# mike-gimelfarb/bboptpy

Measured on AMD Instinct MI355X. Metric: candidate-evals/sec, higher is better.
Workload: dtype f64; 1 GPU; ActiveCMAES n=128 np=4096 rosenbrock, 256 independent populations per GPU in lockstep; populations_per_gpu=256, n=128, np=4096, objective=rosenbrock

## Files before the change

bboptpy_amd/csrc/bbo_cma.hip:

```cpp
#include "bbo_cma_kernels.hpp"
#include "bbo_sep_kernels.hpp"
#include "bbo_eig_mw.hpp"

#include <algorithm>
#include <atomic>
#include <cmath>
#include <cstdlib>
#include <limits>

namespace bbo {

namespace {

enum { K_SAMPLE = 0, K_RANK, K_WHITEN, K_GRAM, K_PATHS, K_COV, K_EIGEN, K_POST, K_STOP, K_COUNT };
static const char *const K_NAMES[K_COUNT] = { "bbo:cma_sample_eval", "bbo:cma_rank", "bbo:cma_whiten", "bbo:cma_gram", "bbo:cma_paths", "bbo:cma_cov", "bbo:cma_eigen", "bbo:cma_post", "bbo:cma_history_stop" };

int pick_maxt(int ld)
{
    const int per_wave = ((ld >> 4) + 3) / 4;
    if (per_wave <= 1) return 1;
    if (per_wave <= 2) return 2;
    if (per_wave <= 4) return 4;
    return 8;
}
// ... 88 lines not shown

bool CmaEngine::mw_reserve(long workgroups)
{
    if (mw_reserved_ == workgroups) return true;
    mw_release();
    if (!MwBudget::get().reserve(params_.device, workgroups)) return false;
    mw_reserved_ = workgroups;
    return true;
}

void CmaEngine::mw_release()
{
    if (mw_reserved_ > 0) MwBudget::get().release(params_.device, mw_reserved_);
    mw_reserved_ = 0;
}

bool CmaEngine::mw_check_failed()
{
    if (!mw_launched_) return false;
    mw_launched_ = false;
    if (!*mw_fail_host_) return false;
    *mw_fail_host_ = 0;
    mw_disabled_ = true;
    mw_release();
    return true;
}

void CmaEngine::set_params(int np, double sigma, int mfev)
{
    params_.np = np;
    params_.sigma0 = sigma;
    params_.mfev = mfev;
    if (params_.bound) {
        params_.bound = 0;
        fprintf(stderr, "Warning [CMA]: box bounding is no longer enabled.\n");
    }
}

void CmaEngine::init(int n, const double *lower, const double *upper, const double *guess,
        const ObjectiveSpec &obj)
{
    const bool sep = params_.algo == BBO_ALGO_SEP_CMAES;
    if (sep)
        BBO_REQUIRE(n >= 1 && n <= 4096, "SepCMAES: dimension must be in [1, 4096]");
    else
        BBO_REQUIRE(n >= 1 && n <= EIG_NMAX, "dimension must be in [1, 512]");
    BBO_HIP(hipSetDevice(params_.device));
    obj_ = obj;
    const int P = params_.populations;
    const int lambda = params_.np;
    CmaConst &c = c_;
    c = CmaConst {};
    c.n = n;
    c.ld = round_up(n, 16);
    c.lambda = lambda;
    c.lambda_pad = round_up(lambda, 16);
    c.mu = lambda / 2;
    c.mu_pad = round_up(c.mu, 16);
    c.variant = sep ? 2 : params_.algo == BBO_ALGO_ACTIVE_CMAES ? 1 : 0;
    c.bound = params_.bound ? 1 : 0;
    c.lazy_isc = (!sep && !c.bound && c.ld > 16 && c.ld <= 256) ? 1 : 0;
    c.obj = obj.on_device() ? obj.builtin : OBJ_HOST;
    c.mfev = params_.mfev;
    c.mit = params_.mfev / lambda;
    c.npop = P;
    c.seed = params_.seed;
    c.tol = params_.tol;
    c.sigma0 = params_.sigma0;
    c.stop_off = 0;
    c.ftarget = -std::numeric_limits<double>::infinity();

    std::vector<double> w(c.mu);
    double sum = 0.;
    for (int i = 0; i < c.mu; i++) {
        w[i] = std::log(0.5 * (lambda + 1.)) - std::log(i + 1.);
        sum += w[i];
    }
    const double inv = 1. / sum;
    for (int i = 0; i < c.mu; i++) w[i] *= inv;
    double lenw = 0.;
    for (int i = 0; i < c.mu; i++) lenw = lenw + w[i] * w[i];
    c.mueff = 1. / lenw;

    c.chi = std::sqrt(n) * (1. - 1. / (4. * n) + 1. / (21. * n * n));
    c.cc = (4. + c.mueff / n) / (n + 4. + 2. * c.mueff / n);
    c.cs = (c.mueff + 2.) / (5. + n + c.mueff);
    c.c1 = 2. / ((1.3 + n) * (1.3 + n) + c.mueff);
    c.cmu = std::min(1. - c.c1,
            2. * (c.mueff - 2. + 1. / c.mueff) / ((2. + n) * (2. + n) + c.mueff));
    c.damps = 1. + c.cs + 2. * std::max(0., std::sqrt((c.mueff - 1.) / (n + 1.)) - 1.);
    c.hlen = 10 + (int) std::ceil((30. * n) / lambda);
    c.ik = (int) std::ceil(0.1 + lambda / 4.);
    c.eigenfreq = params_.eigenrate * lambda / (c.c1 + c.cmu) / n;
    c.cm = 1.;
    c.alphaold = 0.5;
    c.cneg = 0.;
    if (c.variant == 1) {
        const double ac = params_.alphacov;
        c.cc = (4. + 0. * c.mueff / n) / (n + 4. + 0. * 2. * c.mueff / n);
        c.cs = (c.mueff + 2.) / (3. + n + c.mueff);
        c.c1 = ac * std::min(1., lambda / 6.) / ((n + 1.3) * (n + 1.3) + c.mueff);
        c.cmu = 1. - c.c1;
        c.cmu = std::min(c.cmu,
                ac * (c.mueff - 2. + 1. / c.mueff) / ((2. + n) * (2. + n) + ac * c.mueff / 2.));
        c.cneg = (1. - c.cmu) * (ac / 8.) * c.mueff / (std::pow(n + 2., 1.5) + 2. * c.mueff);
        c.damps = 1. + c.cs + 2. * std::max(0., std::sqrt((c.mueff - 1.) / (n + 1.)) - 1.);
        c.eigenfreq = params_.eigenrate * (1. / (c.c1 + c.cmu + c.cneg)) / n;
    }

    if (sep) {
        c.cc = 4. / (n + 4.);
        c.cs = (c.mueff + 2.) / (3. + n + c.mueff);
        c.damps = 1. + c.cs + 2. * std::max(0., std::sqrt((c.mueff - 1.) / (n + 1.)) - 1.);
        c.ccov = 2. / ((n + std::sqrt(2.)) * (n + std::sqrt(2.)) * c.mueff);
        c.ccov += std::min(1., (2. * c.mueff - 1.) / ((n + 2.) * (n + 2.) + c.mueff))
                * (1. - 1. / c.mueff);
        if (params_.adjustlr) c.ccov *= ((n + 2.) / 3.);
    }

    c.rps = 64;
    while (c.rps > 16 && gram_lds_bytes(c.ld, c.rps) > GRAM_LDS_MAX) c.rps >>= 1;
    if (c.ld == 128) {
        int cap = 32;
        if (const char *e = std::getenv("BBO_GRAM_WANT")) cap = std::max(1, std::atoi(e));
        int want = std::max(1, std::min(cap, (512 + P - 1) / P));
        want = std::min(want, (c.lambda_pad + G128_CH - 1) / G128_CH);
        c.rps = ((c.lambda_pad + want - 1) / want + G128_CH - 1) / G128_CH * G128_CH;
    }
    c.splits = (c.lambda_pad + c.rps - 1) / c.rps;
    if (sep)
        c.splits = std::max(1, std::min(c.mu / 16, (1024 + P - 1) / P));

    const size_t ld = c.ld, ld2 = ld * ld;
    const bool same_shape = !sep && keep_bc_ && last_n_ == n && C_.count == P * ld2;
    X_.alloc((size_t) P * c.lambda_pad * ld);
    f_.alloc((size_t) P * c.lambda_pad);
    zn2_.alloc((size_t) P * c.lambda_pad);
    rank_.alloc((size_t) P * c.lambda_pad);
    order_.alloc((size_t) P * c.lambda_pad);
    xmean_.alloc(P * ld);
    xold_.alloc(P * ld);
    pc_.alloc(P * ld);
    ps_.alloc(P * ld);
    D_.alloc(P * ld);
    csep_.alloc(P * ld);
    if (!sep) {
        isc_.alloc(P * ld2);
        BDp_.alloc(P * ld2);
        ISp_.alloc(P * ld2);
    }
    S_.alloc((size_t) P * c.mu_pad);
    gram_part_.alloc((size_t) P * c.splits * (sep ? ld : ld2));
    mean_part_.alloc((size_t) P * c.splits * ld);
    hist_best_.alloc((size_t) P * c.hlen);
    hist_kth_.alloc((size_t) P * c.hlen);
    weights_.alloc(c.mu);
    weights_.upload(w.data(), c.mu);
    lower_.alloc(ld);
    upper_.alloc(ld);
    aux_.alloc(ld);
    scal_.alloc(P);
    zinject_.release();
    zrecord_.release();

    lower_h_.assign(ld, 0.);
    upper_h_.assign(ld, 0.);
    aux_h_.assign(ld, 0.);
    std::copy(lower, lower + n, lower_h_.begin());
    std::copy(upper, upper + n, upper_h_.begin());
    fill_objective_aux(obj.on_device() ? obj.builtin : -1, n, aux_h_.data());
    lower_.upload(lower_h_.data(), ld);
    upper_.upload(upper_h_.data(), ld);
    aux_.upload(aux_h_.data(), ld);

    std::vector<double> eye(sep ? 0 : P * ld2, 0.), ones(P * ld, 1.);
    csep_.upload(ones.data(), P * ld);
    if (!sep) {
    for (int p = 0; p < P; p++)
        for (int i = 0; i < n; i++) eye[p * ld2 + (size_t) i * ld + i] = 1.;
    if (same_shape) {
        std::vector<double> bm(P * ld2), cm(P * ld2);
        B_.download(bm.data(), P * ld2);
        C_.download(cm.data(), P * ld2);
        for (int p = 0; p < P; p++)
            for (int i = 0; i < n; i++) {
                bm[p * ld2 + (size_t) i * ld + i] = 1.;
                cm[p * ld2 + (size_t) i * ld + i] = 1.;
            }
        B_.upload(bm.data(), P * ld2);
        C_.upload(cm.data(), P * ld2);
    } else {
        B_.alloc(P * ld2);
        C_.alloc(P * ld2);
        B_.upload(eye.data(), P * ld2);
        C_.upload(eye.data(), P * ld2);
    }
    isc_.upload(eye.data(), P * ld2);
    }
    D_.upload(ones.data(), P * ld);
    keep_bc_ = !sep;
    last_n_ = n;

    std::vector<double> xm(P * ld, 0.);
    for (int p = 0; p < P; p++) std::copy(guess + (size_t) p * n, guess + (size_t) (p + 1) * n,
            xm.begin() + p * ld);
    xmean_.upload(xm.data(), P * ld);

    std::vector<CmaScal> sc(P);
    for (auto &s : sc) {
        std::memset(&s, 0, sizeof(s));
        s.sigma = params_.sigma0;
        s.fbest = -std::numeric_limits<double>::infinity();
        s.fworst = std::numeric_limits<double>::infinity();
        s.hist_head = -1;
        s.basis_ok = same_shape ? 0 : 1;
    }
    scal_.upload(sc.data(), P);
    basis_maybe_stale_ = same_shape;

    if (!sep) eig_work_.alloc((size_t) P * 4 * eig_slab((int) ld));

    CmaDev &d = d_;
    d = CmaDev {};
    d.X = X_.p; d.f = f_.p; d.rank = rank_.p; d.order = order_.p;
    d.xmean = xmean_.p; d.xold = xold_.p; d.pc = pc_.p; d.ps = ps_.p;
    d.C = C_.p; d.B = B_.p; d.D = D_.p; d.isc = isc_.p; d.BDp = BDp_.p; d.ISp = ISp_.p;
    d.S = S_.p; d.zn2 = zn2_.p; d.csep = csep_.p; d.gram_part = gram_part_.p; d.mean_part = mean_part_.p;
    d.hist_best = hist_best_.p; d.hist_kth = hist_kth_.p; d.eig_work = eig_work_.p;
    d.weights = weights_.p; d.lower = lower_.p; d.upper = upper_.p; d.aux = aux_.p;
    d.zinject = nullptr; d.zrecord = nullptr; d.scal = scal_.p;
    d.stamps = stamps_.p;
    d.mw_fail_host = mw_fail_host_;
    d.mw_fault = mw_fault_from_env();
    mw_release();

    c.honor_stop = 0;
    inited_ = true;
    if (!sep) {
        launch_post(2);
        BBO_HIP(hipGetLastError());
        BBO_HIP(hipStreamSynchronize(stream_));
    }
}

void CmaEngine::launch_post(int mode)
{
    const CmaConst &c = c_;
    if (c.ld <= 128) {
        const size_t lds = (size_t) (c.ld * (c.ld + 2) + c.ld) * sizeof(double);
        allow_lds((const void*) cma_post_mfma<1>, 140 * 1024);
        allow_lds((const void*) cma_post_mfma<4>, 140 * 1024);
        if (c.npop < 32)
            hipLaunchKernelGGL(cma_post_mfma<4>, dim3(c.npop, 4), dim3(256), lds, stream_, d_, c_,
                    mode);
        else
            hipLaunchKernelGGL(cma_post_mfma<1>, dim3(c.npop, 1), dim3(256), lds, stream_, d_, c_,
                    mode);
    } else {
        dim3 grid(c.ld / 16, c.ld / 16, c.npop);
        hipLaunchKernelGGL(cma_post, grid, dim3(256), 0, stream_, d_, c_, mode);
    }
}

void CmaEngine::launch_sample_eval()
{
    const CmaConst &c = c_;
    bool zn_valid = false;
    timer_.begin(stream_, K_SAMPLE);
    if (c.variant == 2) {
        const int per_pop = std::max(1, 4096 / c.npop);
        if (c.ld <= 256) {
            allow_lds((const void*) sep_sample_eval<16>, 128 * 1024);
            const size_t lds = (size_t) 16 * c.ld * sizeof(double);
            hipLaunchKernelGGL(sep_sample_eval<16>,
                    dim3(std::min((c.lambda_pad + 15) / 16, per_pop), c.npop), dim3(256), lds,
                    stream_, d_, c_);
        } else if (c.ld <= 2048) {
            const size_t lds = (size_t) 8 * c.ld * sizeof(double);
            const dim3 grid(std::min((c.lambda_pad + 7) / 8, per_pop), c.npop);
            if (c.n == c.ld && !c.bound && c.lambda == c.lambda_pad && !d_.zinject
                    && !d_.zrecord && !(d_.dbg & 256)) {
                if (sep_sum_objective(c.obj) && !(d_.dbg & 1048576)) {
                    const dim3 sgrid(std::min(c.lambda_pad / (4 * SEP_K), per_pop), c.npop);
#define BBO_SEP_SUM(NCV, OBJV) hipLaunchKernelGGL((sep_sample_sum<256, NCV, OBJV>), sgrid, dim3(256), 0, stream_, d_, c_)
#define BBO_SEP_SUM_OBJ(NCV) \
                    switch (c.obj) { \
                    case OBJ_SPHERE: BBO_SEP_SUM(NCV, OBJ_SPHERE); break; \
                    case OBJ_ELLIPSOID: BBO_SEP_SUM(NCV, OBJ_ELLIPSOID); break; \
                    case OBJ_RASTRIGIN: BBO_SEP_SUM(NCV, OBJ_RASTRIGIN); break; \
                    case OBJ_CIGAR: BBO_SEP_SUM(NCV, OBJ_CIGAR); break; \
                    case OBJ_DISCUS: BBO_SEP_SUM(NCV, OBJ_DISCUS); break; \
                    default: BBO_SEP_SUM(NCV, OBJ_DIFFPOW); break; \
                    }
                    if (c.ld == 1024 && c.obj != OBJ_RASTRIGIN && c.obj != OBJ_DIFFPOW) { BBO_SEP_SUM_OBJ(4) }
                    else { BBO_SEP_SUM_OBJ(0) }
#undef BBO_SEP_SUM_OBJ
#undef BBO_SEP_SUM
                } else {
                    allow_lds((const void*) sep_sample_eval<64, 512, true>, 140 * 1024);
                    hipLaunchKernelGGL((sep_sample_eval<64, 512, true>), grid, dim3(512), lds,
                            stream_, d_, c_);
                }
            } else {
                allow_lds((const void*) sep_sample_eval<64, 512>, 140 * 1024);
                hipLaunchKernelGGL((sep_sample_eval<64, 512>), grid, dim3(512), lds, stream_,
                        d_, c_);
            }
        } else {
            allow_lds((const void*) sep_sample_eval<64>, 140 * 1024);
            const size_t lds = (size_t) 4 * c.ld * sizeof(double);
            hipLaunchKernelGGL(sep_sample_eval<64>,
                    dim3(std::min((c.lambda_pad + 3) / 4, per_pop), c.npop), dim3(256), lds,
                    stream_, d_, c_);
        }
        timer_.end(stream_);
        BBO_HIP(hipGetLastError());
        c_.use_zn = 0;
        return;
    }
    if (c.ld == 128 && (long) c.npop * c.lambda_pad >= sample128_min_rows_
            && (c.obj < 0 || frag_objective_ok(c.obj))) {
        int rw = (int) (((long) c.npop * c.lambda_pad / 256 + 127) / 128) * 128;
        rw = std::max(128, std::min(4096, rw));
        allow_lds((const void*) cma_sample_eval128, 128 * 1024);
        dim3 grid((c.lambda_pad + rw - 1) / rw, c.npop);
        const int full = (c.n == 128 && !c.bound && c.lambda == c.lambda_pad && !d_.zinject
                && !d_.zrecord && !(d_.dbg & 256)) ? 1 : 0;
        hipLaunchKernelGGL(cma_sample_eval128, grid, dim3(512), 128 * 1024, stream_, d_, c_, rw,
                full);
        zn_valid = true;
    } else if (c.ld == 128 && (long) c.npop * (c.lambda_pad / 16) <= sample_wide_max_tiles_) {
        const size_t lds = (size_t) 16 * (c.ld + 2) * sizeof(double);
        hipLaunchKernelGGL((cma_sample_eval<1, 8>), dim3(c.lambda_pad / 16, c.npop), dim3(512), lds, stream_,
                d_, c_);
        zn_valid = true;
    } else if (c.ld <= 128) {
        dim3 grid((c.lambda_pad + 63) / 64, c.npop);
        const size_t lds = (size_t) 64 * (c.ld + 2) * sizeof(double);
        allow_lds((const void*) cma_sample_eval64<1>, 80 * 1024);
        allow_lds((const void*) cma_sample_eval64<2>, 80 * 1024);
        if (c.ld <= 32)
            hipLaunchKernelGGL((cma_sample_eval64<1, 8>), grid, dim3(256), lds, stream_, d_, c_);
        else if (c.ld <= 64)
            hipLaunchKernelGGL(cma_sample_eval64<1>, grid, dim3(256), lds, stream_, d_, c_);
        else
            hipLaunchKernelGGL(cma_sample_eval64<2>, grid, dim3(256), lds, stream_, d_, c_);
        zn_valid = true;
    } else {
        dim3 grid(c.lambda_pad / 16, c.npop);
        const size_t lds = (size_t) 16 * (c.ld + 2) * sizeof(double);
        allow_lds((const void*) cma_sample_eval<8>, 80 * 1024);
        if ((long) grid.x * grid.y <= 32 && c.ld <= 256 && !(d_.dbg & 268435456))
            hipLaunchKernelGGL((cma_sample_eval<1, 16>), grid, dim3(1024), lds, stream_, d_, c_);
        else
        switch (pick_maxt(c.ld)) {
        case 1: hipLaunchKernelGGL(cma_sample_eval<1>, grid, dim3(256), lds, stream_, d_, c_); break;
        case 2: hipLaunchKernelGGL(cma_sample_eval<2>, grid, dim3(256), lds, stream_, d_, c_); break;
        case 4: hipLaunchKernelGGL(cma_sample_eval<4>, grid, dim3(256), lds, stream_, d_, c_); break;
        default: hipLaunchKernelGGL(cma_sample_eval<8>, grid, dim3(256), lds, stream_, d_, c_); break;
        }
        zn_valid = true;
    }
    timer_.end(stream_);
    BBO_HIP(hipGetLastError());
    c_.use_zn = (zn_valid && !c.bound) ? 1 : 0;
}

void CmaEngine::launch_rank()
{
    const CmaConst &c = c_;
    rank_wrote_norms_ = false;
    timer_.begin(stream_, K_RANK);
    if (c.lambda <= 64 && c.lambda >= 2 && c.npop >= 4) {
        hipLaunchKernelGGL(cma_rank_wave, dim3((c.npop + 3) / 4), dim3(256), 0, stream_, d_, c_);
    } else if (c.lambda <= SORT_LDS_MAX && c.npop >= 4) {
        int m = 2;
        while (m < c.lambda) m <<= 1;
        allow_lds((const void*) cma_rank_sort, 128 * 1024);
        const size_t lds = rank_sort_merges(m, d_.dbg) ? (size_t) m * 24 : (size_t) std::max(m, 1024) * 12;
        hipLaunchKernelGGL(cma_rank_sort, dim3(c.npop), dim3(sort_threads(m)), lds, stream_, d_,
                c_, m);
        rank_wrote_norms_ = c.variant == 1 && c.use_zn && !basis_maybe_stale_;
    } else {
        if ((long) c.npop * ((c.lambda + 31) / 32) <= 256 && c.lambda >= 2048 && !(d_.dbg & (128 | 4096)))
            hipLaunchKernelGGL(cma_rank64, dim3((c.lambda + 3) / 4, c.npop), dim3(256), 0, stream_, d_, c_);
        else if ((long) c.npop * ((c.lambda + 31) / 32) <= 512 && c.lambda >= 512 && !(d_.dbg & 128))
            hipLaunchKernelGGL(cma_rank32, dim3((c.lambda + 7) / 8, c.npop), dim3(256), 0, stream_, d_, c_);
        else
            hipLaunchKernelGGL(cma_rank, dim3((c.lambda + 31) / 32, c.npop), dim3(256), 0, stream_, d_, c_);
        rank_wrote_norms_ = c.variant == 1 && c.use_zn && !basis_maybe_stale_;
    }
    timer_.end(stream_);
    BBO_HIP(hipGetLastError());
}

void CmaEngine::launch_update()
{
    const CmaConst &c = c_;
    if (c.variant == 2) {
        timer_.begin(stream_, K_GRAM);
        hipLaunchKernelGGL(sep_moments, dim3(c.splits, (c.ld + 511) / 512, c.npop), dim3(256), 0,
                stream_, d_, c_);
        timer_.end(stream_);
        timer_.begin(stream_, K_PATHS);
        hipLaunchKernelGGL(sep_paths, dim3(c.npop), dim3(256), 0, stream_, d_, c_);
        timer_.end(stream_);
        BBO_HIP(hipGetLastError());
        return;
    }
    const bool norms_done = rank_wrote_norms_;
    rank_wrote_norms_ = false;
    if (c.variant == 1 && !norms_done) {
        timer_.begin(stream_, K_WHITEN);
        if (c.ld == 128 && (long) c.npop * c.mu_pad >= 256 * 128) {
            int rw = (int) (((long) c.npop * c.mu_pad / 256 + 127) / 128) * 128;
            rw = std::max(128, std::min(2048, rw));
            const size_t lds = (size_t) (128 * 128 + 128) * sizeof(double);
            allow_lds((const void*) cma_whiten128, 132 * 1024);
            dim3 grid128((c.mu_pad + rw - 1) / rw, c.npop);
            hipLaunchKernelGGL(cma_whiten128, grid128, dim3(512), lds, stream_, d_, c_, rw);
        } else {
        dim3 grid(c.mu_pad / 16, c.npop);
        const size_t lds = (size_t) (16 * (c.ld + 2) + 64) * sizeof(double);
        allow_lds((const void*) cma_whiten<8>, 80 * 1024);
        switch (pick_maxt(c.ld)) {
        case 1: hipLaunchKernelGGL(cma_whiten<1>, grid, dim3(256), lds, stream_, d_, c_); break;
        case 2: hipLaunchKernelGGL(cma_whiten<2>, grid, dim3(256), lds, stream_, d_, c_); break;
        case 4: hipLaunchKernelGGL(cma_whiten<4>, grid, dim3(256), lds, stream_, d_, c_); break;
        default: hipLaunchKernelGGL(cma_whiten<8>, grid, dim3(256), lds, stream_, d_, c_); break;
        }
        }
        timer_.end(stream_);
        BBO_HIP(hipGetLastError());
    }
    if (c.ld == 128) {
        const size_t lds = (size_t) (2 * G128_CH * G128_LDY + 4 * G128_CH) * sizeof(double);
        allow_lds((const void*) cma_gram128, 80 * 1024);
        timer_.begin(stream_, K_GRAM);
        if (d_.dbg & 512)
            hipLaunchKernelGGL(cma_gram128, dim3(c.splits, c.npop), dim3(256), lds, stream_, d_, c_);
        else
            hipLaunchKernelGGL(cma_gram128s, dim3(c.splits, c.npop), dim3(256), 0, stream_, d_, c_);
        timer_.end(stream_);
        BBO_HIP(hipGetLastError());
    } else {
        const int NT = c.ld / 16, LT = NT * (NT + 1) / 2;
        const int ldy = gram_ldy(c.ld);
        dim3 grid(c.splits, (LT + 4 * GRAM_TPW - 1) / (4 * GRAM_TPW), c.npop);
        const size_t lds = gram_lds_bytes(c.ld, c.rps);
        allow_lds((const void*) cma_gram, (int) GRAM_LDS_MAX);
        timer_.begin(stream_, K_GRAM);
        hipLaunchKernelGGL(cma_gram, grid, dim3(256), lds, stream_, d_, c_, ldy);
        timer_.end(stream_);
        BBO_HIP(hipGetLastError());
    }
    timer_.begin(stream_, K_PATHS);
    if (c.lazy_isc && c.n >= 64 && !(d_.dbg & 131072))
        hipLaunchKernelGGL(cma_paths_lazy1k, dim3(c.npop), dim3(1024), 0, stream_, d_, c_);
    else if (c.lazy_isc)
        hipLaunchKernelGGL(cma_paths_lazy, dim3(c.npop), dim3(256), 0, stream_, d_, c_);
    else
        hipLaunchKernelGGL(cma_paths, dim3(c.npop), dim3(256), 0, stream_, d_, c_);
    timer_.end(stream_);
    BBO_HIP(hipGetLastError());
    {
        const int total = c.n * (c.n + 1) / 2;
        dim3 grid((total + 255) / 256, c.npop);
        timer_.begin(stream_, K_COV);
        hipLaunchKernelGGL(cma_cov, grid, dim3(256), 0, stream_, d_, c_);
        timer_.end(stream_);
        BBO_HIP(hipGetLastError());
    }
}

int CmaEngine::next_mw_xcd()
{
    static std::atomic<int> counter { 0 };
    return counter.fetch_add(1) & 7;
}

void CmaEngine::launch_eigen()
{
    const CmaConst &c = c_;
    if (c.variant == 2) return;
    const EigPlan pl_lds = eig_plan(c.n, c.ld);
    const bool split128 = pl_lds.use_lds && pl_lds.threads == 512 && pl_lds.dc && c.npop <= split_maxp_
            && !(d_.dbg & (2 | 4 | 8 | 1024 | 4194304));
    const EigPlan pl = split128 ? eig_plan_split(c.n, c.ld) : pl_lds;
    bool wy4_packs = false, fcols_closed = false;
    allow_lds((const void*) cma_eigen, 160 * 1024 - 768);
    allow_lds((const void*) cma_eigen_g, 160 * 1024 - 768);
    allow_lds((const void*) cma_eigen_b, 160 * 1024 - 768);
    allow_lds((const void*) cma_eigen_256, 160 * 1024 - 768);
    allow_lds((const void*) cma_eigen_128, 160 * 1024 - 768);
    timer_.begin(stream_, K_EIGEN);
    const bool big_spread = c.n > 256 && pl.dc && !pl.hybrid && !mw_disabled_
            && !(d_.dbg & (2 | 16777216)) && mw_reserve((long) c.npop * 16);
    const bool small = c.n <= 16 && c.n >= 2 && c.ld == 16 && !(d_.dbg & 16);
    if (small)
        hipLaunchKernelGGL(cma_eigen_small, dim3((c.npop + 3) / 4), dim3(256), 0, stream_, d_, c_, 0,
                1);
    else if (pl.threads == 128)
        hipLaunchKernelGGL(cma_eigen_128, dim3(c.npop), dim3(128), pl.lds_bytes, stream_, d_, c_,
                pl, 0);
    else if (pl.threads == 256)
        hipLaunchKernelGGL(cma_eigen_256, dim3(c.npop), dim3(256), pl.lds_bytes, stream_, d_, c_,
                pl, 0);
    else if (pl.use_lds)
        hipLaunchKernelGGL(cma_eigen, dim3(c.npop), dim3(512), pl.lds_bytes, stream_, d_, c_,
                pl, 0);
    else if (pl.hybrid && !(d_.dbg & (2 | 1024 | 4194304))) {
        const EigPlan plh = eig_plan(128, 128);
        allow_lds((const void*) cma_eigen_g1, 160 * 1024 - 768);
        allow_lds((const void*) cma_eigen_g2, 160 * 1024 - 768);
        allow_lds((const void*) cma_eig_halves, 160 * 1024 - 768);
        const bool use_mw = !split128 && !mw_disabled_ && !(d_.dbg & 16777216) && mw_reserve((long) c.npop * MW_G);
        if (split128) {
            allow_lds((const void*) cma_eigen_r1, 160 * 1024 - 768);
            hipLaunchKernelGGL(cma_eigen_r1, dim3(c.npop), dim3(512), pl_lds.lds_bytes, stream_, d_, c_,
                    pl_lds, 0);
        } else if (use_mw) {
            mw_launched_ = true;
            if (mw_buf_.count != (size_t) c.npop * MW_BUF_DOUBLES) mw_buf_.alloc((size_t) c.npop * MW_BUF_DOUBLES);
            const int istop = (d_.dbg & 536870912) ? 1 : 128;
            hipLaunchKernelGGL(cma_tred_mw, dim3(8 * MW_G, c.npop), dim3(MW_T), 0, stream_, d_, c_, 0,
                    mw_buf_.p, ++mw_launch_, istop, mw_xcd_);
            if (istop > 1) {
                allow_lds((const void*) cma_tred_tail, 160 * 1024 - 768);
                hipLaunchKernelGGL(cma_tred_tail, dim3(c.npop), dim3(512), pl.lds_bytes, stream_, d_, c_, pl, 0);
            }
        } else
        hipLaunchKernelGGL(cma_eigen_g1, dim3(c.npop), dim3(512), pl.lds_bytes, stream_, d_, c_, pl, 0);
        hipLaunchKernelGGL(cma_eig_halves, dim3(3, c.npop), dim3(512), plh.lds_bytes, stream_, d_, c_,
                plh, pl.lda);
        if ((long) c.npop * 8 <= 256 && !(d_.dbg & 67108864)) {
            hipLaunchKernelGGL(cma_eigen_g2, dim3(c.npop), dim3(512), pl.lds_bytes, stream_, d_, c_, pl, 1);
            hipLaunchKernelGGL(cma_eig_secular, dim3((c.n + 31) / 32, c.npop), dim3(512), 0, stream_, d_, c_);
            fcols_closed = !(c.n & 1) && c.lazy_isc && (long) c.npop * ((c.n + 15) / 16) <= 256
                    && !(d_.dbg & (33554432 | 134217728));
            if (fcols_closed) {
                hipLaunchKernelGGL(cma_eig_lowner, dim3((c.n + 31) / 32, c.npop), dim3(512), 0, stream_, d_, c_);
                hipLaunchKernelGGL(cma_eig_fcols, dim3((c.n + 31) / 32, c.npop), dim3(512), 0, stream_, d_, c_);
            } else
            hipLaunchKernelGGL(cma_eigen_g2, dim3(c.npop), dim3(512), pl.lds_bytes, stream_, d_, c_, pl, 2);
        } else
        hipLaunchKernelGGL(cma_eigen_g2, dim3(c.npop), dim3(512), pl.lds_bytes, stream_, d_, c_, pl, 0);
    } else if (pl.hybrid)
        hipLaunchKernelGGL(cma_eigen_g, dim3(c.npop), dim3(512), pl.lds_bytes, stream_, d_, c_,
                pl, 0);
    else if (big_spread) {
        const bool chain = !(d_.dbg & 536870912);
        mw_launched_ = true;
        const size_t need = (size_t) c.npop * (mw_buf_doubles(512) + mw_buf_doubles(256));
        if (mw_buf_.count != need) mw_buf_.alloc(need);
        hipLaunchKernelGGL(cma_tred_mw512, dim3(8 * 16, c.npop), dim3(MW_T), 0, stream_, d_, c_, 0,
                mw_buf_.p, ++mw_launch_, chain ? 256 : 128, mw_xcd_);
        if (chain)
            hipLaunchKernelGGL(cma_tred_mw_chain, dim3(8 * MW_G, c.npop), dim3(MW_T), 0, stream_, d_, c_,
                    mw_buf_.p + (size_t) c.npop * mw_buf_doubles(512), ++mw_launch_, 128, mw_xcd_);
        const EigPlan plt = eig_plan(256, 256);
        allow_lds((const void*) cma_tred_tail, 160 * 1024 - 768);
        hipLaunchKernelGGL(cma_tred_tail, dim3(c.npop), dim3(512), plt.lds_bytes, stream_, d_, c_, plt,
                chain ? 1 : 0);
        allow_lds((const void*) cma_eigen_b4, 160 * 1024 - 768);
        hipLaunchKernelGGL(cma_eigen_b4, dim3(c.npop), dim3(512), pl.lds_bytes, stream_, d_, c_, pl, 0);
    } else
        hipLaunchKernelGGL(cma_eigen_b, dim3(c.npop), dim3(512), pl.lds_bytes, stream_, d_, c_,
                pl, 0);
    timer_.end(stream_);
    BBO_HIP(hipGetLastError());
    if (pl.dc && !pl.reg_path && (pl.hybrid || !(d_.dbg & 2))) {
        dim3 grid((c.n + 63) / 64, (c.n + 63) / 64, c.npop);
        const bool narrow = (long) grid.x * grid.y * grid.z < 128;
        dim3 grid1((c.n + 15) / 16, (c.n + 63) / 64, c.npop);
        if (narrow)
            hipLaunchKernelGGL(cma_eig_gemm1, grid1, dim3(256), 0, stream_, d_, c_, pl.lda, 0);
        else
            hipLaunchKernelGGL(cma_eig_gemm, grid, dim3(256), 0, stream_, d_, c_, pl.lda, 0);
        if (big_spread)
            hipLaunchKernelGGL(cma_eig_wy4_512, dim3((c.n + 15) / 16, c.npop), dim3(256), 0, stream_, d_, c_);
        else if ((d_.dbg & 2) || !pl.hybrid)
            hipLaunchKernelGGL(cma_eig_gemm, grid, dim3(256), 0, stream_, d_, c_, pl.lda, 1);
        else
        {
            if ((long) c.npop * ((c.n + 15) / 16) <= 256 && !(d_.dbg & 134217728)) {
                wy4_packs = c.lazy_isc != 0;
                hipLaunchKernelGGL(cma_eig_wy4, dim3((c.n + 15) / 16, c.npop), dim3(256), 0, stream_, d_, c_,
                        wy4_packs ? (fcols_closed ? 2 : 1) : 0);
            } else
            hipLaunchKernelGGL(cma_eig_wy, dim3((c.n + 63) / 64, c.npop), dim3(256), 0, stream_, d_,
                    c_);
        }
        BBO_HIP(hipGetLastError());
    }
    timer_.begin(stream_, K_POST);
// ... 519 lines not shown
```

bboptpy_amd/csrc/bbo_cma.hpp:

```cpp
#pragma once

#include "bbo_common.hpp"

namespace bbo {

struct CmaScal {
    double sigma;
    double fbest, fworst;
    double pslen;
    double ybw[4];
    int ibw[4];
    int it, fev;
    int flag;
    int stop;
    int hsig;
    int eigenlastev, eigen_done;
    int hist_head, hist_len;
    int basis_ok;
    int eig_stage;
    int eig_mw_fail;
};

struct CmaConst {
    int n, ld;
    int lambda, lambda_pad;
    int mu, mu_pad;
    int variant;
    int bound, obj;
    int use_zn;
    int lazy_isc;
    int mfev, mit, hlen, ik;
    int honor_stop;
    int splits, rps;
    int npop;
    double mueff, cc, cs, c1, cmu, cneg, alphaold, cm, damps, chi, sigma0, tol, eigenfreq;
    double ccov;
    uint64_t seed;
    int stop_off;
    double ftarget;
};

struct CmaDev {
    double *X;
    double *f;
    int *rank;
    int *order;
    double *xmean, *xold, *pc, *ps;
    double *C;
    double *B;
    double *D;
    double *isc;
    double *BDp;
    double *ISp;
    double *S;
    double *csep;
    double *zn2;
    double *gram_part;
    double *mean_part;
    double *hist_best, *hist_kth;
    double *eig_work;
    const double *weights;
    const double *lower, *upper, *aux;
    const double *zinject;
    double *zrecord;
    CmaScal *scal;
    long long *stamps;
    int dbg;
    int mw_fault;
    int *mw_fail_host;
};

class CmaEngine: public Optimizer {
public:
    explicit CmaEngine(const bbo_params &p);
    ~CmaEngine() override;

    void init(int n, const double *lower, const double *upper, const double *guess,
            const ObjectiveSpec &obj) override;
    void iterate() override;
    void solution(int population, double *x_out, int *n_evals, int *converged) override;
    void optimize(int n, const double *lower, const double *upper, const double *guess,
            const ObjectiveSpec &obj, double *x_out, int *n_evals, int *converged) override;
    int run(int max_generations) override;
    int get(const std::string &key, int population, double *out, int cap) override;
    int set(const std::string &key, int population, const double *in, int count) override;
    int dimension() const override { return c_.n; }

    void set_params(int np, double sigma, int mfev);
    void phase(int which);
    void inject_normals(const double *z, int count);
    double evaluate_point(const double *x);
    int lambda() const { return params_.np; }
    int populations() const { return params_.populations; }
    uint64_t seed() const { return params_.seed; }
    void set_seed(uint64_t s) { params_.seed = s; }
    void fresh_start(uint64_t s)
    {
        params_.seed = s;
        keep_bc_ = false;
    }

private:
    void generation(bool honor_stop);
    bool small_fused_ok() const;
    void launch_small(int gens, bool honor_stop);
    void launch_sample_eval();
    void launch_post(int mode);
    void launch_rank();
    void launch_update();
    void launch_eigen();
    void launch_history_stop();
    void host_evaluate();
    void fetch_scal(std::vector<CmaScal> &out);
    bool all_stopped();

    bbo_params params_;
    ObjectiveSpec obj_;
    CmaConst c_ {};
    CmaDev d_ {};
    hipStream_t stream_ = nullptr;
    bool inited_ = false;
    bool keep_bc_ = false;
    bool basis_maybe_stale_ = false;
    DevBuf<double> mw_buf_;
    unsigned long long mw_launch_ = 0;
    bool mw_disabled_ = false;
    int mw_xcd_ = next_mw_xcd();
    static int next_mw_xcd();
    long sample_wide_max_tiles_ = 512;
    long sample128_min_rows_ = 256 * 128;
    int split_maxp_ = 32;
    bool rank_wrote_norms_ = false;
    int last_n_ = -1;
    std::vector<double> lower_h_, upper_h_, aux_h_;

    DevBuf<double> zn2_, csep_;
    DevBuf<double> X_, f_, xmean_, xold_, pc_, ps_, C_, B_, D_, isc_, BDp_, ISp_, S_,
            gram_part_, mean_part_, hist_best_, hist_kth_, eig_work_, weights_, lower_,
            upper_, aux_, zinject_, zrecord_;
    DevBuf<int> rank_, order_;
    DevBuf<long long> stamps_;
    DevBuf<CmaScal> scal_;
    int *mw_fail_host_ = nullptr;
    long mw_reserved_ = 0;
    bool mw_launched_ = false;
    bool mw_reserve(long workgroups);
    void mw_release();
    bool mw_check_failed();
    KernelTimer timer_;
};

}
```

bboptpy_amd/csrc/bbo_cma_kernels.hpp:

```cpp
#pragma once

#include "bbo_cma.hpp"
#include "bbo_objectives.hpp"
#include "bbo_rng.hpp"
#include "bbo_eig.hpp"
#include "bbo_rank.hpp"

namespace bbo {

typedef double d4_t __attribute__((ext_vector_type(4)));

#define BBO_INF (__builtin_huge_val())

__device__ inline double wave_sum(double v)
{
#pragma unroll
    for (int off = 32; off > 0; off >>= 1) v += __shfl_xor(v, off, 64);
    return v;
}

__device__ inline void cma_wave_sync()
{
    __builtin_amdgcn_fence(__ATOMIC_SEQ_CST, "wavefront");
    __builtin_amdgcn_wave_barrier();
// ... 1034 lines not shown
        case 0: gram128_chunk<0>(Y[buf], V[buf], W[buf], acc, macc, fr, fk); break;
        case 1: gram128_chunk<1>(Y[buf], V[buf], W[buf], acc, macc, fr, fk); break;
        case 2: gram128_chunk<2>(Y[buf], V[buf], W[buf], acc, macc, fr, fk); break;
        default: gram128_chunk<3>(Y[buf], V[buf], W[buf], acc, macc, fr, fk); break;
        }
        if (ch + 1 < nch) stash(ch + 1, buf ^ 1);
        __syncthreads();
    }

    double *G = d.gram_part + ((size_t) p * c.splits + s) * 128 * 128;
    double *mp = d.mean_part + ((size_t) p * c.splits + s) * 128;
    switch (wave) {
    case 0: gram128_store<0>(G, mp, acc, macc, lane, isig); break;
    case 1: gram128_store<1>(G, mp, acc, macc, lane, isig); break;
    case 2: gram128_store<2>(G, mp, acc, macc, lane, isig); break;
    default: gram128_store<3>(G, mp, acc, macc, lane, isig); break;
    }
}

template<int WV>
__device__ __forceinline__ void gram128_stream(const CmaDev &d, const CmaConst &c, int p, int s,
        double *coef, int lane)
{
    const CmaScal *sc = d.scal + p;
    const double *Xp = d.X + (size_t) p * c.lambda_pad * 128;
    const double *xold = d.xmean + (size_t) p * 128;
    const int *rank = d.rank + (size_t) p * c.lambda_pad;
    const double isig = 1. / sc->sigma;
    const int row0 = s * c.rps;
    const int nrows = min(c.rps, c.lambda_pad - row0);
    const int nch = (nrows + G128_CH - 1) / G128_CH;
    const int fr = lane & 15, fk = lane >> 4;
    const bool pace = !(d.dbg & 65536);

    double xo[8];
#pragma unroll
    for (int i = 0; i < 8; i++) xo[i] = g128_needs_y(WV, i) ? xold[16 * i + fr] : 0.;
    d4_t acc[9];
    double macc[8];
#pragma unroll
    for (int t = 0; t < 9; t++) acc[t] = d4_t { 0., 0., 0., 0. };
#pragma unroll
    for (int i = 0; i < 8; i++) macc[i] = 0.;

    double ring[4][8];
    const int lane_off = fk * 128 + fr;
    auto load_step = [&](int ch, int ks, int slot) {
        const int blk = min(row0 + ch * G128_CH + 4 * ks, c.lambda_pad - 4);
        const double *src = Xp + (size_t) blk * 128;
#pragma unroll
        for (int i = 0; i < 8; i++)
            if (g128_needs_y(WV, i)) ring[slot][i] = src[lane_off + 16 * i];
    };
    const double cmu1 = c.variant == 1 ? c.cmu + c.cneg * (1. - c.alphaold) : c.cmu;
    const double *Sp = d.S + (size_t) p * c.mu_pad;
    int rk = 0;
    int rk2 = 0;
    double wa = 0., sk = 1., sm = 1.;
    auto coef_link1 = [&](int ch) {
        const int row = row0 + ch * G128_CH + lane;
        const bool ok = lane < G128_CH && ch < nch && row < c.lambda;
        rk = rank[ok ? row : 0];
        if (!ok) rk = -1;
    };
    auto coef_link2 = [&]() {
        rk2 = rk;
        const bool pos = rk2 >= 0 && rk2 < c.mu;
        const int k = min(max(c.lambda - 1 - rk2, 0), c.mu - 1);
        wa = d.weights[pos ? rk2 : k];
        sk = Sp[k];
        sm = Sp[c.mu - 1 - k];
    };
    auto put_coef = [&](int buf) {
        double pv = 0., pw = 0.;
        if (rk2 >= 0 && rk2 < c.mu) {
            pw = wa;
            pv = cmu1 * wa;
        } else if (rk2 >= 0 && c.variant == 1 && rk2 >= c.lambda - c.mu) {
            const double ycoeff = sk / fmax(sm, 1e-8);
            pv = -c.cneg * wa * ycoeff;
        }
        if (lane < G128_CH) {
            coef[buf * 2 * G128_CH + lane] = pv;
            coef[buf * 2 * G128_CH + G128_CH + lane] = pw;
        }
    };
    auto sweep_step = [&](int slot, double vk, double wk) {
        double y[8], a[8];
#pragma unroll
        for (int i = 0; i < 8; i++) {
            y[i] = a[i] = 0.;
            if (g128_needs_y(WV, i)) y[i] = ring[slot][i] - xo[i];
            if (g128_needs_a(WV, i)) a[i] = vk * y[i];
        }
        if (WV == 1 || WV == 2) {
#pragma unroll
            for (int i = 0; i < 8; i++)
                if (g128_mean(WV, i)) macc[i] = fma(wk, y[i], macc[i]);
        }
#pragma unroll
        for (int t = 0; t < 9; t++)
            acc[t] = __builtin_amdgcn_mfma_f64_16x16x4f64(a[G128_TI[WV][t]], y[G128_TJ[WV][t]],
                    acc[t], 0, 0, 0);
    };

    coef_link1(0);
    coef_link2();
    put_coef(0);
    coef_link1(1);
    coef_link2();
    coef_link1(2);
#pragma unroll
    for (int ks = 0; ks < 4; ks++) load_step(0, ks, ks);
    cma_wave_sync();
    for (int ch = 0; ch < nch; ch++) {
        const int buf = ch & 1;
        double vk = coef[buf * 2 * G128_CH + fk], wk = coef[buf * 2 * G128_CH + G128_CH + fk];
#pragma unroll
        for (int ks = 0; ks < 8; ks++) {
            double vn = 0., wn = 0.;
            if (ks < 7) {
                vn = coef[buf * 2 * G128_CH + 4 * (ks + 1) + fk];
                if (WV == 1 || WV == 2) wn = coef[buf * 2 * G128_CH + G128_CH + 4 * (ks + 1) + fk];
            }
            sweep_step(ks & 3, vk, wk);
            vk = vn;
            wk = wn;
            if (ks < 4) load_step(ch, ks + 4, ks & 3);
            else load_step(ch + 1, ks - 4, ks & 3);
            __builtin_amdgcn_sched_barrier(0);
        }
        put_coef(buf ^ 1);
        coef_link2();
        coef_link1(ch + 3);
        cma_wave_sync();
        if (pace && (ch & (G128_PACE - 1)) == G128_PACE - 1) __builtin_amdgcn_s_barrier();
    }
    double *G = d.gram_part + ((size_t) p * c.splits + s) * 128 * 128;
    double *mp = d.mean_part + ((size_t) p * c.splits + s) * 128;
    gram128_store<WV>(G, mp, acc, macc, lane, isig);
}

__global__ __launch_bounds__(256, 2) void cma_gram128s(CmaDev d, CmaConst c)
{
    const int p = blockIdx.y, s = blockIdx.x;
    if (pop_frozen(c, d.scal + p)) return;
    __shared__ double coef[4][2 * 2 * G128_CH];
    const int lane = threadIdx.x & 63, wave = threadIdx.x >> 6;
    switch (wave) {
    case 0: gram128_stream<0>(d, c, p, s, coef[0], lane); break;
    case 1: gram128_stream<1>(d, c, p, s, coef[1], lane); break;
    case 2: gram128_stream<2>(d, c, p, s, coef[2], lane); break;
    default: gram128_stream<3>(d, c, p, s, coef[3], lane); break;
    }
}

template<bool LAZY = false, int T = 256>
__device__ __forceinline__ void paths_body(const CmaDev &d, const CmaConst &c, int p)
{
    CmaScal *sc = d.scal + p;
    if (pop_frozen(c, sc)) return;
    __shared__ double dm[512];
    __shared__ double red[T / 64];
    const int tid = threadIdx.x, ld = c.ld;
    double *xmean = d.xmean + (size_t) p * ld, *xold = d.xold + (size_t) p * ld;
    double *ps = d.ps + (size_t) p * ld, *pc = d.pc + (size_t) p * ld;
    const double sigma = sc->sigma;

    for (int j = tid; j < ld; j += T) {
        double sum = 0.;
        {
            const double *mp = d.mean_part + (size_t) p * c.splits * ld + j;
            int s = 0;
            for (; s + 8 <= c.splits; s += 8) {
                double x[8];
#pragma unroll
                for (int u = 0; u < 8; u++) x[u] = mp[(size_t) (s + u) * ld];
                __builtin_amdgcn_sched_barrier(0);
#pragma unroll
                for (int u = 0; u < 8; u++) sum += x[u];
            }
            for (; s < c.splits; s++) sum += mp[(size_t) s * ld];
        }
        const double xo = xmean[j];
        sum = xo + sigma * sum;
        double xn = 0.;
        if (j < c.n) {
            xn = c.variant == 1 ? xo * (1. - c.cm) + sum * c.cm : sum;
            if (c.bound) xn = fmax(d.lower[j], fmin(xn, d.upper[j]));
        }
        xold[j] = xo;
        xmean[j] = xn;
        dm[j] = xn - xo;
    }
    __syncthreads();

    const double csc = sqrt(c.cs * (2. - c.cs) * c.mueff);
    const double den = c.variant == 1 ? c.cm * sigma : sigma;
    const double *isc = d.isc + (size_t) p * ld * ld;
    double ssq = 0.;
    if (LAZY && sc->basis_ok) {
        constexpr int HN = T / 128;
        constexpr int RS = T / 16, NU = 128 / RS;
        __shared__ double sv[256], cv[256], part[HN - 1][128];
        const double *B = d.B + (size_t) p * ld * ld, *D = d.D + (size_t) p * ld;
        for (int jb = 0; jb < c.n; jb += 128) {
            const int j = jb + (tid & 127), h = tid >> 7;
            double t0 = 0., t1 = 0., t2 = 0., t3 = 0.;
            if (j < c.n) {
                int i = h;
                for (; i + 7 * HN < c.n; i += 8 * HN) {
                    double b[8];
#pragma unroll
                    for (int u = 0; u < 8; u++) b[u] = B[(size_t) (i + HN * u) * ld + j];
                    t0 += b[0] * dm[i] + b[4] * dm[i + 4 * HN];
                    t1 += b[1] * dm[i + HN] + b[5] * dm[i + 5 * HN];
                    t2 += b[2] * dm[i + 2 * HN] + b[6] * dm[i + 6 * HN];
                    t3 += b[3] * dm[i + 3 * HN] + b[7] * dm[i + 7 * HN];
                }
                for (; i < c.n; i += HN) t0 += B[(size_t) i * ld + j] * dm[i];
            }
            const double t = (t0 + t1) + (t2 + t3);
            if (h > 0) part[h - 1][tid & 127] = t;
            __syncthreads();
            if (h == 0) {
                double tt = t;
#pragma unroll
                for (int q = 0; q < HN - 1; q++) tt += part[q][tid & 127];
                sv[j] = j < c.n ? tt / D[j] : 0.;
            }
            __syncthreads();
        }
        for (int ib = 0; ib < c.n; ib += 128) {
            const int g = tid & 15, r = ib + (tid >> 4);
            double a[NU];
#pragma unroll
            for (int u = 0; u < NU; u++) {
                const int i = r + RS * u;
                double tot = 0.;
                for (int kb = 0; kb < c.n; kb += 128) {
                    double x[8];
#pragma unroll
                    for (int k = 0; k < 8; k++) {
                        const int j = kb + g + 16 * k;
                        x[k] = (i < c.n && j < c.n) ? B[(size_t) i * ld + j] * sv[j] : 0.;
                    }
                    const double part8 = ((x[0] + x[1]) + (x[2] + x[3])) + ((x[4] + x[5]) + (x[6] + x[7]));
                    tot = kb == 0 ? part8 : tot + part8;
                }
                a[u] = tot;
            }
#pragma unroll
            for (int u = 0; u < NU; u++) {
                const double v = group_sum<16>(a[u]);
                if (g == 0 && r + RS * u < c.n) cv[r + RS * u] = v;
            }
        }
        __syncthreads();
        for (int i = tid; i < ld; i += T) {
            const double v = i < c.n ? (1. - c.cs) * ps[i] + csc * cv[i] / den : 0.;
            ps[i] = v;
            ssq += v * v;
        }
    } else {
        for (int i = tid; i < ld; i += T) {
            double v = 0.;
            if (i < c.n) {
                double acc = 0.;
                for (int j = 0; j < c.n; j++) acc += isc[(size_t) j * ld + i] * dm[j];
                v = (1. - c.cs) * ps[i] + csc * acc / den;
            }
            ps[i] = v;
            ssq += v * v;
        }
    }
    ssq = wave_sum(ssq);
    if ((tid & 63) == 0) red[tid >> 6] = ssq;
    __syncthreads();
    double rsum = 0.;
#pragma unroll
    for (int q = 0; q < T / 64; q++) rsum += red[q];
    const double pslen = sqrt(rsum);

    const double denom = 1. - pow(1. - c.cs, 2. * sc->fev / c.lambda);
    const int hsig = (pslen / sqrt(denom) / c.chi < 1.4 + 2. / (c.n + 1.)) ? 1 : 0;

    const double ccc = sqrt(c.cc * (2. - c.cc) * c.mueff);
    for (int i = tid; i < ld; i += T) {
        double v = 0.;
        if (i < c.n) v = (1. - c.cc) * pc[i] + hsig * ccc * dm[i] / den;
        pc[i] = v;
    }

    if (tid == 0) {
        const double *f = d.f + (size_t) p * c.lambda_pad;
        const int *order = d.order + (size_t) p * c.lambda_pad;
        double sg = sigma * exp(fmin(1., (c.cs / c.damps) * (pslen / c.chi - 1.)));
        if (f[order[0]] == f[order[c.ik]]) sg *= exp(0.2 + c.cs / c.damps);
        if (sc->it >= c.hlen && sc->fworst - sc->fbest == 0.) sg *= exp(0.2 + c.cs / c.damps);
        sc->sigma = sg;
        sc->hsig = hsig;
        sc->pslen = pslen;
    }
}

__global__ __launch_bounds__(256) void cma_paths(CmaDev d, CmaConst c)
// ... 583 lines not shown
```

Baseline: 683.9 million candidate-evals/s.

## Add ring-buffered direct-to-LDS gram kernel for n=128 with async global loads

Adds a new default gram kernel for ld=128 that streams sample rows into a 4-deep LDS ring buffer using global_load_lds async copies with counted vmcnt waits. Each wave issues its share of upcoming stages while MFMA sweeps consume the current one. Rank coefficients are precomputed into a new global table and also async-loaded per stage. The aim is to hide global memory latency behind the f64 MFMA accumulation. The cost is more LDS per block, which may reduce occupancy, and fragile hand-written waitcnt and barrier logic. The previous streaming kernel stays available behind a debug flag.

```diff
diff --git a/bboptpy_amd/csrc/bbo_cma.hip b/bboptpy_amd/csrc/bbo_cma.hip
--- a/bboptpy_amd/csrc/bbo_cma.hip
+++ b/bboptpy_amd/csrc/bbo_cma.hip
@@ -264,6 +264,7 @@
     S_.alloc((size_t) P * c.mu_pad);
     gram_part_.alloc((size_t) P * c.splits * (sep ? ld : ld2));
     mean_part_.alloc((size_t) P * c.splits * ld);
+    gcoef_.alloc(ld == 128 ? (size_t) P * c.lambda_pad * 2 : 0);
     hist_best_.alloc((size_t) P * c.hlen);
     hist_kth_.alloc((size_t) P * c.hlen);
     weights_.alloc(c.mu);
@@ -338,6 +339,7 @@
     d.xmean = xmean_.p; d.xold = xold_.p; d.pc = pc_.p; d.ps = ps_.p;
     d.C = C_.p; d.B = B_.p; d.D = D_.p; d.isc = isc_.p; d.BDp = BDp_.p; d.ISp = ISp_.p;
     d.S = S_.p; d.zn2 = zn2_.p; d.csep = csep_.p; d.gram_part = gram_part_.p; d.mean_part = mean_part_.p;
+    d.gcoef = gcoef_.p;
     d.hist_best = hist_best_.p; d.hist_kth = hist_kth_.p; d.eig_work = eig_work_.p;
     d.weights = weights_.p; d.lower = lower_.p; d.upper = upper_.p; d.aux = aux_.p;
     d.zinject = nullptr; d.zrecord = nullptr; d.scal = scal_.p;
@@ -549,10 +551,13 @@
         const size_t lds = (size_t) (2 * G128_CH * G128_LDY + 4 * G128_CH) * sizeof(double);
         allow_lds((const void*) cma_gram128, 80 * 1024);
         timer_.begin(stream_, K_GRAM);
+        allow_lds((const void*) cma_gram128l, G128L_LDS);
         if (d_.dbg & 512)
             hipLaunchKernelGGL(cma_gram128, dim3(c.splits, c.npop), dim3(256), lds, stream_, d_, c_);
+        else if (d_.dbg & 2097152)
+            hipLaunchKernelGGL(cma_gram128s, dim3(c.splits, c.npop), dim3(256), 0, stream_, d_, c_);
         else
-            hipLaunchKernelGGL(cma_gram128s, dim3(c.splits, c.npop), dim3(256), 0, stream_, d_, c_);
+            hipLaunchKernelGGL(cma_gram128l, dim3(c.splits, c.npop), dim3(256), G128L_LDS, stream_, d_, c_);
         timer_.end(stream_);
         BBO_HIP(hipGetLastError());
     } else {
diff --git a/bboptpy_amd/csrc/bbo_cma.hpp b/bboptpy_amd/csrc/bbo_cma.hpp
--- a/bboptpy_amd/csrc/bbo_cma.hpp
+++ b/bboptpy_amd/csrc/bbo_cma.hpp
@@ -57,6 +57,7 @@
     double *zn2;
     double *gram_part;
     double *mean_part;
+    double *gcoef;
     double *hist_best, *hist_kth;
     double *eig_work;
     const double *weights;
@@ -136,7 +137,7 @@
 
     DevBuf<double> zn2_, csep_;
     DevBuf<double> X_, f_, xmean_, xold_, pc_, ps_, C_, B_, D_, isc_, BDp_, ISp_, S_,
-            gram_part_, mean_part_, hist_best_, hist_kth_, eig_work_, weights_, lower_,
+            gram_part_, mean_part_, gcoef_, hist_best_, hist_kth_, eig_work_, weights_, lower_,
             upper_, aux_, zinject_, zrecord_;
     DevBuf<int> rank_, order_;
     DevBuf<long long> stamps_;
diff --git a/bboptpy_amd/csrc/bbo_cma_kernels.hpp b/bboptpy_amd/csrc/bbo_cma_kernels.hpp
--- a/bboptpy_amd/csrc/bbo_cma_kernels.hpp
+++ b/bboptpy_amd/csrc/bbo_cma_kernels.hpp
@@ -1210,6 +1210,139 @@
     case 1: gram128_stream<1>(d, c, p, s, coef[1], lane); break;
     case 2: gram128_stream<2>(d, c, p, s, coef[2], lane); break;
     default: gram128_stream<3>(d, c, p, s, coef[3], lane); break;
+    }
+}
+
+constexpr int G128L_RS = 16;
+constexpr int G128L_D = 4;
+constexpr int G128L_LDS = (G128L_D * G128L_RS * G128_LDY + G128L_D * G128L_RS * 2) * (int) sizeof(double);
+
+typedef __attribute__((address_space(1))) void g128l_gvoid;
+typedef __attribute__((address_space(3))) void g128l_lvoid;
+
+template<int N>
+__device__ __forceinline__ void g128l_wait_barrier()
+{
+    asm volatile("s_waitcnt vmcnt(%0) lgkmcnt(0)" :: "n"(N) : "memory");
+    __builtin_amdgcn_s_barrier();
+    asm volatile("" ::: "memory");
+}
+
+template<int WV>
+__device__ __forceinline__ void gram128_ring(const CmaDev &d, const CmaConst &c, int p, int s,
+        double *lds)
+{
+    constexpr int D = G128L_D, RS = G128L_RS;
+    constexpr int L = RS / 4 + (WV == 0);
+    double *Y = lds;
+    double *VW = lds + D * RS * G128_LDY;
+    const CmaScal *sc = d.scal + p;
+    const double *Xp = d.X + (size_t) p * c.lambda_pad * 128;
+    const double *xold = d.xmean + (size_t) p * 128;
+    const int *rank = d.rank + (size_t) p * c.lambda_pad;
+    double *tab = d.gcoef + (size_t) p * c.lambda_pad * 2;
+    const int tid = threadIdx.x, lane = tid & 63, fr = lane & 15, fk = lane >> 4;
+    const double isig = 1. / sc->sigma;
+    const int row0 = s * c.rps;
+    const int nst = min(c.rps, c.lambda_pad - row0) / RS;
+
+    auto issue_rows = [&](int st) {
+        double *dst = Y + (st & (D - 1)) * RS * G128_LDY;
+        const double *src = Xp + (size_t) (row0 + st * RS) * 128 + 2 * lane;
+#pragma unroll
+        for (int j = 0; j < RS / 4; j++) {
+            const int r = (RS / 4) * WV + j;
+            __builtin_amdgcn_global_load_lds((g128l_gvoid*) (src + r * 128), (g128l_lvoid*) (dst + r * G128_LDY),
+                    16, 0, 0);
+        }
+    };
+    auto issue_coef = [&](int st) {
+        if (WV == 0)
+            __builtin_amdgcn_global_load_lds(
+                    (g128l_gvoid*) (reinterpret_cast<const float*>(tab + 2 * (row0 + st * RS)) + lane),
+                    (g128l_lvoid*) (VW + (st & (D - 1)) * RS * 2), 4, 0, 0);
+    };
+
+    double xo[8];
+#pragma unroll
+    for (int i = 0; i < 8; i++) xo[i] = g128_needs_y(WV, i) ? xold[16 * i + fr] : 0.;
+    const int pre = min(nst, D - 1);
+    for (int st = 0; st < pre; st++) issue_rows(st);
+    for (int r = tid; r < nst * RS; r += 256) {
+        const int row = row0 + r;
+        double wm = 0., vg = 0.;
+        if (row < c.lambda) rank_coefficients(d, c, p, rank[row], wm, vg);
+        *reinterpret_cast<double2*>(&tab[2 * row]) = make_double2(vg, wm);
+        if (r < pre * RS) *reinterpret_cast<double2*>(&VW[2 * r]) = make_double2(vg, wm);
+    }
+    asm volatile("s_waitcnt vmcnt(0)" ::: "memory");
+    __syncthreads();
+
+    d4_t acc[9];
+    double macc[8];
+#pragma unroll
+    for (int t = 0; t < 9; t++) acc[t] = d4_t { 0., 0., 0., 0. };
+#pragma unroll
+    for (int i = 0; i < 8; i++) macc[i] = 0.;
+
+    auto sweep = [&](int buf) {
+        const double *Yb = Y + buf * RS * G128_LDY + fr;
+        const double *Vb = VW + buf * RS * 2;
+#pragma unroll
+        for (int ks = 0; ks < RS / 4; ks++) {
+            const int k = 4 * ks + fk;
+            const double vk = Vb[2 * k];
+            double y[8], a[8];
+#pragma unroll
+            for (int i = 0; i < 8; i++) {
+                y[i] = a[i] = 0.;
+                if (g128_needs_y(WV, i)) y[i] = Yb[k * G128_LDY + 16 * i] - xo[i];
+                if (g128_needs_a(WV, i)) a[i] = vk * y[i];
+            }
+            if (WV == 1 || WV == 2) {
+                const double wk = Vb[2 * k + 1];
+#pragma unroll
+                for (int i = 0; i < 8; i++)
+                    if (g128_mean(WV, i)) macc[i] = fma(wk, y[i], macc[i]);
+            }
+#pragma unroll
+            for (int t = 0; t < 9; t++)
+                acc[t] = __builtin_amdgcn_mfma_f64_16x16x4f64(a[G128_TI[WV][t]], y[G128_TJ[WV][t]],
+                        acc[t], 0, 0, 0);
+        }
+    };
+
+    int st = 0;
+    for (; st + D - 1 < nst; st++) {
+        g128l_wait_barrier<(D - 2) * L>();
+        issue_rows(st + D - 1);
+        issue_coef(st + D - 1);
+        sweep(st & (D - 1));
+    }
+    for (; st < nst; st++) {
+        switch (nst - 1 - st) {
+        case 2: g128l_wait_barrier<2 * L>(); break;
+        case 1: g128l_wait_barrier<L>(); break;
+        default: g128l_wait_barrier<0>(); break;
+        }
+        sweep(st & (D - 1));
+    }
+    double *G = d.gram_part + ((size_t) p * c.splits + s) * 128 * 128;
+    double *mp = d.mean_part + ((size_t) p * c.splits + s) * 128;
+    gram128_store<WV>(G, mp, acc, macc, lane, isig);
+}
+
+__global__ __launch_bounds__(256, 2) void cma_gram128l(CmaDev d, CmaConst c)
+{
+    static_assert(G128L_D == 4, "the tail's counted waits assume two stages behind the oldest");
+    const int p = blockIdx.y, s = blockIdx.x;
+    if (pop_frozen(c, d.scal + p)) return;
+    extern __shared__ __attribute__((aligned(16))) double lds[];
+    switch (threadIdx.x >> 6) {
+    case 0: gram128_ring<0>(d, c, p, s, lds); break;
+    case 1: gram128_ring<1>(d, c, p, s, lds); break;
+    case 2: gram128_ring<2>(d, c, p, s, lds); break;
+    default: gram128_ring<3>(d, c, p, s, lds); break;
     }
 }
 
```

Result: no change. 685.8 million candidate-evals/s, median of 6 (+0.3%).
